# HSU-ANT/gstpeaq

Measured on AMD Instinct MI355X. Metric: 2048-sample stereo ref/test frame-pairs/sec (basic PEAQ, ear model -> MOVs -> ODG); ODG delta vs CPU ref, higher is better.
Workload: dtype f64

## Files before the change

### gstpeaq_amd/csrc/peaq_backend.hip

```cpp
#include <hip/hip_runtime.h>

#include <climits>
#include <cstdlib>

#include "peaq_device.h"
#include "peaq_kernels.h"
#include "peaq_wave.h"
#ifdef PEAQ_DEV_PROBES
#define PEAQ_DEV_TU_BACKEND
#include "dev_probes.inc"
#endif
#ifndef PEAQ_DEV_SPIN_INSTEAD_OF_BACKEND
#define PEAQ_DEV_SPIN_INSTEAD_OF_BACKEND(a, block, stream)
#endif

namespace peaq {

constexpr int kLdsBands = 128;
constexpr int kPaPad = 4, kPaStride = kPaPad + kLdsBands + 4;

constexpr int kAccLdsStride = 16;
struct LaneAcc {
  double* f;
  int mode, status;
// ... 299 lines not shown
            ld *
            (bt.pow(1. + div_fast(fmax(stest * e_test[s] - sref * e_ref[s], 0.), ethres + sref * e_ref[s] * beta), 0.23) - 1.);
        nl += t;
        terms[s] = t;
      }
    }
  }
  return nl;
}
template <int NB>
__device__ __forceinline__ double noise_loudness_total(double sum, double nl_min) {
  const double nl = sum * (24. / NB);
  return nl < nl_min ? 0. : nl;
}

template <int NB, int SLOTS, class TAB, bool TERMS = false>
__device__ __forceinline__ void mod_difference(const BandLane<NB, SLOTS>& bl, const TAB& bt,
                                               double lev_wt, const double (&mr)[SLOTS], const double (&mt)[SLOTS],
                                               const double (&loud_ref)[SLOTS], double& d1, double& d2, double& wt,
                                               double (*terms)[SLOTS] = nullptr) {
  double a1 = 0., a2 = 0., aw = 0.;
#pragma unroll
  for (int s = 0; s < SLOTS; ++s) {
    if (TERMS) terms[0][s] = terms[1][s] = terms[2][s] = 0.;
    if (bl.valid(s)) {
      const double diff = fabs(mr[s] - mt[s]);
      if (!TERMS) {
        a1 += div_fast(diff, 1. + mr[s]);
        a2 += div_fast((mt[s] >= mr[s] ? 1. : .1) * diff, 0.01 + mr[s]);
        aw += div_fast(loud_ref[s], loud_ref[s] + lev_wt * bt.noise_pow03(bl.band(s)));
      } else {
        a1 += terms[0][s] = div_fast(diff, 1. + mr[s]);
        a2 += terms[1][s] = div_fast((mt[s] >= mr[s] ? 1. : .1) * diff, 0.01 + mr[s]);
        aw += terms[2][s] = div_fast(loud_ref[s], loud_ref[s] + lev_wt * bt.noise_pow03(bl.band(s)));
      }
    }
  }
  double unused;
  wave_sum4(a1, a2, aw, 0., d1, d2, wt, unused);
}

__device__ __forceinline__ uint32_t wave_uniform(uint32_t x) { return (uint32_t)__builtin_amdgcn_readfirstlane((int)x); }
template <bool FB>
struct PointWalk {
  PointSnap* row;
  uint32_t n_min, interval;
  int n_points, k;
  uint32_t due;
  __device__ __forceinline__ static uint32_t count(uint32_t a) {
    return FB ? a / kFbFrame : a >= (uint32_t)kFrame ? (a - kFrame) / kHop + 1 : 0u;
  }
  __device__ __forceinline__ void set_due(int k1) {
    k = k1;
    if (k1 >= n_points) {
      due = UINT_MAX;
      return;
    }
    const uint64_t t = (uint64_t)(k1 + 1) * interval;
    due = count(t < n_min ? (uint32_t)t : n_min);
  }
  __device__ __forceinline__ void init(const PointArgs& p, unsigned pair, uint32_t c0) {
    row = p.snap + (size_t)pair * p.n_points;
    const uint32_t nr = p.n_ref ? p.n_ref[pair] : p.n_uniform, nt = p.n_test ? p.n_test[pair] : p.n_uniform;
    n_min = nr < nt ? nr : nt;
    interval = p.interval;
    n_points = p.n_points;
    const uint64_t thr = FB ? (uint64_t)kFbFrame * (c0 + 1ull) : (uint64_t)kFrame + (uint64_t)kHop * c0;
    const uint64_t k0 = n_min < thr ? (uint64_t)n_points : (thr + interval - 1) / interval - 1;
    set_due(k0 < (uint64_t)n_points ? (int)k0 : n_points);
  }
  __device__ __forceinline__ PointSnap* take(uint32_t c) {
    if (wave_uniform(due) != c) return nullptr;
    const int k1 = (int)wave_uniform((uint32_t)k);
    const uint64_t r = reinterpret_cast<uint64_t>(row);
    PointSnap* sp = reinterpret_cast<PointSnap*>(((uint64_t)wave_uniform((uint32_t)(r >> 32)) << 32) |
                                                 wave_uniform((uint32_t)r)) + k1;
    set_due(k1 + 1);
    return sp;
  }
};

template <int NB, class ARGS>
__device__ __forceinline__ void band_store(const ARGS& bnd, uint32_t bit, size_t cell, int lane, double v0, double v1) {
  if (!(bnd.planes & bit)) return;
  const unsigned n_planes = __builtin_popcount(bnd.planes), slot = __builtin_popcount(bnd.planes & (bit - 1u));
  char* __restrict__ row = reinterpret_cast<char*>(bnd.bands + (cell * n_planes + slot) * band_row(NB));
  unsigned off = (unsigned)lane * 16u;
  asm volatile("" : "+v"(off));
  if (2 * lane < NB) *reinterpret_cast<double2*>(row + off) = make_double2(v0, v1);
}

__device__ __forceinline__ void fb_band_store(const FbBandArgs& bnd, uint32_t bit, size_t row0, int lane, double v) {
  if (!(bnd.planes & bit)) return;
  const unsigned slot = __builtin_popcount(bnd.planes & (bit - 1u));
  char* __restrict__ row = reinterpret_cast<char*>(bnd.bands + (row0 + slot) * kFbBands);
  unsigned off = (unsigned)lane * 8u;
  asm volatile("" : "+v"(off));
  if (lane < kFbBands) *reinterpret_cast<double*>(row + off) = v;
}

__device__ __forceinline__ double fb_summary_pick(int lane, double band_value, double den) {
  return lane < kFbBands ? band_value : lane == kFbBands ? den : 0.;
}
__device__ __forceinline__ void fb_summary_add(double* entry, bool own, double v) {
  if (own) *entry += v;
}
__device__ __forceinline__ void fb_summary_copy(double* dst, const double* src, bool own) {
  if (!own) return;
#pragma unroll
  for (int k = 0; k < kFbSumRows; ++k) {
    asm volatile("" ::: "memory");
    dst[k * kFbSumRow] = src[k * kFbSumRow];
  }
}

__device__ __forceinline__ void summary_add(double* row, bool own, double v0, double v1) {
  if (!own) return;
  double2* __restrict__ p = reinterpret_cast<double2*>(row);
  double2 v = *p;
  v.x += v0;
  v.y += v1;
  *p = v;
}
__device__ __forceinline__ void summary_max(double* row, bool own, bool last, double v0, double v1) {
  if (!own) return;
  double2* __restrict__ p = reinterpret_cast<double2*>(row);
  double2 v = *p;
  if (v0 > v.x) v.x = v0;
  if (last)
    v.y += 1.;
  else if (v1 > v.y)
    v.y = v1;
  *p = v;
}
template <int R, int ROW>
__device__ __forceinline__ void summary_copy(double* dst, const double* src, bool own) {
  if (!own) return;
#pragma unroll
  for (int k = 0; k < R; ++k) {
    asm volatile("" ::: "memory");
    *reinterpret_cast<double2*>(dst + k * ROW) = *reinterpret_cast<const double2*>(src + k * ROW);
  }
}

enum { MB_BW_REF, MB_BW_TEST, MB_NMR, MB_WINMOD, MB_ADB, MB_EHS, MB_AVGMOD1, MB_AVGMOD2, MB_NOISELOUD, MB_MFPD,
       MB_RELDIST };
enum { MA_RMSMOD, MA_NLASYM, MA_SEGNMR, MA_EHS, MA_LINDIST };

struct BackendShared {
  double pa[2][2][kPaStride];
  double pc[2][kLdsBands];
  double qc[2][kLdsBands];
  double acc[2][kAccFields][kAccLdsStride];
  double energy[2];
  int gate[2];
};

template <int NB, bool ADV, bool DBG = false>
__global__ __launch_bounds__(128, 3) void backend_kernel(BackendArgs a) {
  constexpr bool PTS = false, TRC = false, BND = false, PBD = false, SUM = false;
  constexpr SummaryArgs sum{};
  constexpr PointArgs pts{};
  constexpr TraceArgs trc{};
  constexpr BandArgs bnd{};
  constexpr PatternBandArgs pbd{};
#include "peaq_backend_fft.inc"
}
template <int NB, bool ADV>
__global__ __launch_bounds__(128, 3) void backend_points_kernel(BackendArgs a, PointArgs pts) {
  constexpr bool DBG = false, PTS = true, TRC = false, BND = false, PBD = false, SUM = false;
  constexpr SummaryArgs sum{};
  constexpr TraceArgs trc{};
  constexpr BandArgs bnd{};
  constexpr PatternBandArgs pbd{};
#include "peaq_backend_fft.inc"
}
template <int NB, bool ADV>
__global__ __launch_bounds__(128, 3) void backend_trace_kernel(BackendArgs a, TraceArgs trc) {
  constexpr bool DBG = false, PTS = false, TRC = true, BND = false, PBD = false, SUM = false;
  constexpr SummaryArgs sum{};
  constexpr PointArgs pts{};
  constexpr BandArgs bnd{};
  constexpr PatternBandArgs pbd{};
#include "peaq_backend_fft.inc"
}
template <int NB, bool ADV>
__global__ __launch_bounds__(128, 3) void backend_bands_kernel(BackendArgs a, BandArgs bnd) {
  constexpr bool DBG = false, PTS = false, TRC = false, BND = true, PBD = false, SUM = false;
  constexpr SummaryArgs sum{};
  constexpr PointArgs pts{};
  constexpr TraceArgs trc{};
  constexpr PatternBandArgs pbd{};
#include "peaq_backend_fft.inc"
}
template <int NB, bool ADV>
__global__ __launch_bounds__(128, 3) void backend_pattern_bands_kernel(BackendArgs a, PatternBandArgs pbd) {
  static_assert(!ADV, "the 55-band path has no pattern layer");
  constexpr bool DBG = false, PTS = false, TRC = false, BND = false, PBD = true, SUM = false;
  constexpr SummaryArgs sum{};
  constexpr PointArgs pts{};
  constexpr TraceArgs trc{};
  constexpr BandArgs bnd{};
#include "peaq_backend_fft.inc"
}
template <int NB, bool ADV>
__global__ __launch_bounds__(128, 3) void backend_summary_kernel(BackendArgs a, SummaryArgs sum) {
  constexpr bool DBG = false, PTS = false, TRC = false, BND = false, PBD = false, SUM = true;
  constexpr PointArgs pts{};
  constexpr TraceArgs trc{};
  constexpr BandArgs bnd{};
  constexpr PatternBandArgs pbd{};
#include "peaq_backend_fft.inc"
}

hipError_t launch_backend(const BackendArgs& a, unsigned n_pairs, hipStream_t stream, const RunOutputs& out) {
  if (n_pairs == 0) return hipSuccess;
  const dim3 block(64 * a.channels);
  PEAQ_DEV_SPIN_INSTEAD_OF_BACKEND(a, block, stream)
  const bool pts = out.has_pts(), trc = out.has_trc(), bnd = out.has_bnd(), pbd = out.has_pbd(), sum = out.has_sum();
  const int alone = bnd + pbd + sum;
  if (alone && (alone + pts + trc + (a.debug != nullptr) + (a.pair_frame0 != nullptr) > 1 || (pbd && a.advanced) ||
                (sum && a.pair_slot)))
    return hipErrorInvalidValue;
  if (out.has_win() && (!trc || alone || pts || a.debug || a.pair_frame0 || a.pair_slot || a.advanced))
    return hipErrorInvalidValue;
  if (sum && !a.advanced)
    hipLaunchKernelGGL((backend_summary_kernel<109, false>), dim3(n_pairs), block, 0, stream, a, out.sum);
  else if (sum)
    hipLaunchKernelGGL((backend_summary_kernel<55, true>), dim3(n_pairs), block, 0, stream, a, out.sum);
  else if (pbd)
    hipLaunchKernelGGL((backend_pattern_bands_kernel<109, false>), dim3(n_pairs), block, 0, stream, a, out.pbd);
  else if (bnd && !a.advanced)
    hipLaunchKernelGGL((backend_bands_kernel<109, false>), dim3(n_pairs), block, 0, stream, a, out.bnd);
  else if (bnd)
    hipLaunchKernelGGL((backend_bands_kernel<55, true>), dim3(n_pairs), block, 0, stream, a, out.bnd);
  else if (trc && !a.advanced)
    hipLaunchKernelGGL((backend_trace_kernel<109, false>), dim3(n_pairs), block, 0, stream, a, out.trc);
  else if (trc)
    hipLaunchKernelGGL((backend_trace_kernel<55, true>), dim3(n_pairs), block, 0, stream, a, out.trc);
  else if (pts && !a.advanced)
    hipLaunchKernelGGL((backend_points_kernel<109, false>), dim3(n_pairs), block, 0, stream, a, out.pts);
  else if (pts)
    hipLaunchKernelGGL((backend_points_kernel<55, true>), dim3(n_pairs), block, 0, stream, a, out.pts);
  else if (!a.advanced && a.debug)
    hipLaunchKernelGGL((backend_kernel<109, false, true>), dim3(n_pairs), block, 0, stream, a);
  else if (a.debug)
    hipLaunchKernelGGL((backend_kernel<55, true, true>), dim3(n_pairs), block, 0, stream, a);
  else if (!a.advanced)
    hipLaunchKernelGGL((backend_kernel<109, false>), dim3(n_pairs), block, 0, stream, a);
  else
    hipLaunchKernelGGL((backend_kernel<55, true>), dim3(n_pairs), block, 0, stream, a);
  return hipGetLastError();
}

struct FbBackendShared {
  double pa[2][2][kPaStride];
  double acc[2][kAccFields][kAccLdsStride];
  int gate[2];
};

template <bool DBG>
__global__ __launch_bounds__(128, 4) void fb_backend_kernel(FbBackendArgs a) {
  constexpr bool PTS = false, TRC = false, BND = false, FSUM = false;
  constexpr PointArgs pts{};
  constexpr TraceArgs trc{};
  constexpr FbBandArgs bnd{};
  constexpr FbSummaryArgs fsum{};
#include "peaq_backend_fb.inc"
}
__global__ __launch_bounds__(128, 4) void fb_backend_points_kernel(FbBackendArgs a, PointArgs pts) {
  constexpr bool DBG = false, PTS = true, TRC = false, BND = false, FSUM = false;
  constexpr TraceArgs trc{};
  constexpr FbBandArgs bnd{};
  constexpr FbSummaryArgs fsum{};
#include "peaq_backend_fb.inc"
}
__global__ __launch_bounds__(128, 4) void fb_backend_trace_kernel(FbBackendArgs a, TraceArgs trc) {
  constexpr bool DBG = false, PTS = false, TRC = true, BND = false, FSUM = false;
  constexpr PointArgs pts{};
  constexpr FbBandArgs bnd{};
  constexpr FbSummaryArgs fsum{};
#include "peaq_backend_fb.inc"
}
__global__ __launch_bounds__(128, 4) void fb_backend_bands_kernel(FbBackendArgs a, FbBandArgs bnd) {
  constexpr bool DBG = false, PTS = false, TRC = false, BND = true, FSUM = false;
  constexpr PointArgs pts{};
  constexpr TraceArgs trc{};
  constexpr FbSummaryArgs fsum{};
#include "peaq_backend_fb.inc"
}
__global__ __launch_bounds__(128, 4) void fb_band_summary_kernel(FbBackendArgs a, FbSummaryArgs fsum) {
  constexpr bool DBG = false, PTS = false, TRC = false, BND = false, FSUM = true;
  constexpr PointArgs pts{};
  constexpr TraceArgs trc{};
  constexpr FbBandArgs bnd{};
#include "peaq_backend_fb.inc"
}

hipError_t launch_fb_backend(const FbBackendArgs& a, unsigned n_pairs, hipStream_t stream, const RunOutputs& out) {
  if (n_pairs == 0) return hipSuccess;
  const bool pts = out.has_pts(), trc = out.has_trc(), bnd = out.has_fbnd(), fsum = out.has_fsum();
  if ((bnd || fsum) && (pts || trc || a.debug || a.windows || (bnd && fsum) || (fsum && out.has_sum())))
    return hipErrorInvalidValue;
  if (fsum)
    hipLaunchKernelGGL(fb_band_summary_kernel, dim3(n_pairs), dim3(64 * a.channels), 0, stream, a, out.fsum);
  else if (bnd)
    hipLaunchKernelGGL(fb_backend_bands_kernel, dim3(n_pairs), dim3(64 * a.channels), 0, stream, a, out.fbnd);
  else if (trc)
    hipLaunchKernelGGL(fb_backend_trace_kernel, dim3(n_pairs), dim3(64 * a.channels), 0, stream, a, out.trc);
  else if (pts)
    hipLaunchKernelGGL(fb_backend_points_kernel, dim3(n_pairs), dim3(64 * a.channels), 0, stream, a, out.pts);
  else if (a.debug)
    hipLaunchKernelGGL(fb_backend_kernel<true>, dim3(n_pairs), dim3(64 * a.channels), 0, stream, a);
  else
    hipLaunchKernelGGL(fb_backend_kernel<false>, dim3(n_pairs), dim3(64 * a.channels), 0, stream, a);
  return hipGetLastError();
}

__global__ void state_init_kernel(PairState* st, unsigned n_pairs) {
  const unsigned pair = blockIdx.x;
  if (pair >= n_pairs) return;
  PairState* ps = st + pair;
  double* raw = reinterpret_cast<double*>(ps);
  for (unsigned i = threadIdx.x; i < sizeof(PairState) / sizeof(double); i += blockDim.x) raw[i] = 0.;
  __syncthreads();
  if (threadIdx.x == 0) {
    ps->loudness_reached = UINT_MAX;
    for (int i = 0; i < kMaxAcc; ++i) ps->status[i] = kInit;
    for (int c = 0; c < 2; ++c)
      for (int i = 0; i < kMaxAcc; ++i) {
        ps->ch[c].acc[i][3] = ps->ch[c].acc[i][4] = ps->ch[c].acc[i][5] = __builtin_nan("");
      }
  }
}

hipError_t launch_state_init(PairState* state, int , unsigned n_pairs, hipStream_t stream) {
  if (n_pairs == 0) return hipSuccess;
  hipLaunchKernelGGL(state_init_kernel, dim3(n_pairs), dim3(256), 0, stream, state, n_pairs);
  return hipGetLastError();
}

static_assert(kInit == 0, "points_init_kernel writes status as zero");
__global__ void points_init_kernel(double* __restrict__ raw, size_t n_doubles) {
  const size_t i = (size_t)blockIdx.x * blockDim.x + threadIdx.x;
  if (i >= n_doubles) return;
  const unsigned j = (unsigned)(i % kSnapDoubles);
  double v = 0.;
  if (j >= (unsigned)kSnapAccHead) {
    const unsigned f = (j - kSnapAccHead) % kAccFields;
    if (f >= 3 && f <= 5) v = __builtin_nan("");
  }
  raw[i] = v;
}

hipError_t launch_points_init(PointSnap* snap, size_t n_snaps, hipStream_t stream) {
  if (n_snaps == 0) return hipSuccess;
  const size_t n = n_snaps * kSnapDoubles;
  hipLaunchKernelGGL(points_init_kernel, dim3((unsigned)((n + 255) / 256)), dim3(256), 0, stream,
                     reinterpret_cast<double*>(snap), n);
  return hipGetLastError();
// ... 129 lines not shown
```

### gstpeaq_amd/csrc/peaq_backend_fft.inc

```
  __shared__ BackendShared sh;
  __shared__ double sh_tab[T_COUNT * kBandStride];
  __shared__ __attribute__((aligned(16))) double sh_ltab[2 * kLogTabEntries + 2];
  constexpr int SLOTS = 2;
  const int lane = threadIdx.x & 63;
  const int chan = __builtin_amdgcn_readfirstlane(threadIdx.x >> 6);
  const int channels = a.channels;
  const unsigned pair = blockIdx.x;
  const BandLane<NB, SLOTS> bl{lane};
  {
    const BandTables* __restrict__ g = a.bands;
    const double* const src[T_COUNT] = {g->adapt_tc, g->ear_tc, g->threshold, g->loud_factor, g->exc_threshold,
                                        g->internal_noise, g->noise_pow03, g->mask_diff, g->inv_spread_norm,
                                        g->inv_spread_norm_pow03, g->ln_internal_noise, g->inv_window_count};
#pragma unroll
    for (int t = 0; t < T_COUNT; ++t)
      for (int i = threadIdx.x; i < kBandStride; i += blockDim.x) sh_tab[t * kBandStride + i] = src[t][i];
    for (int i = threadIdx.x; i < 2 * kLogTabEntries; i += blockDim.x) sh_ltab[i] = a.common->log_tab[i >> 1][i & 1];
  }
  LdsTabs bt{sh_tab, 0, a.bands->deriv_factor, sh_ltab};
  PairState* __restrict__ ps = a.state + (a.pair_slot ? a.pair_slot[pair] : pair);
  ChannelState* __restrict__ cs = &ps->ch[chan];

  unsigned f_begin, f_end;
  if (a.pair_frame0) {
    f_begin = a.pair_frame0[pair];
    f_end = f_begin + a.pair_nframes[pair];
  } else {
    const unsigned n_frames = a.n_frames ? a.n_frames[pair] : a.n_frames_uniform;
    f_begin = a.frame0;
    f_end = a.frame0 + a.frames_per_launch;
    if (f_end > n_frames) f_end = n_frames;
  }
  if (f_begin >= f_end) return;
  const bool clk_wave = a.clk && blockIdx.x == 0 && chan == 0;
  unsigned long long clk_s0 = 0, clk_w0 = 0;
  if (clk_wave) {
    clk_w0 = wall_clock64();
    clk_s0 = __builtin_readcyclecounter();
  }
  if (lane < kPaPad) sh.pa[chan][0][lane] = sh.pa[chan][1][lane] = 0.;
  __syncthreads();

  constexpr int SUM_R = band_summary_rows(ADV), SUM_ROW = band_row(NB);
  __shared__ __attribute__((aligned(16))) double sh_sum[SUM ? 2 * SUM_R * SUM_ROW : 2];
  const bool sum_own = SUM && 2 * lane < NB;
  const bool sum_last = SUM && 2 * lane + 1 == NB;
  auto sum_at = [&](double* base) -> double* {
    unsigned off = (unsigned)lane * 16u;
    asm volatile("" : "+v"(off));
    return reinterpret_cast<double*>(reinterpret_cast<char*>(base) + off);
  };
  auto sum_row = [&](int k) -> double* { return sum_at(sh_sum + (SUM ? (chan * SUM_R + k) * SUM_ROW : 0)); };
  auto sum_cell = [&](double* base) -> double* {
    return sum_at(base + ((size_t)pair * channels + chan) * (SUM_R * SUM_ROW));
  };
  int sum_st = kInit;
  if (SUM) {
    sum_st = __builtin_amdgcn_readfirstlane(ps->status[ADV ? (int)MA_SEGNMR : (int)MB_NMR]);
    summary_copy<SUM_R, SUM_ROW>(sum_row(0), sum_cell(sum.rows), sum_own);
  }

  double sm[2][SLOTS];
  double la[6][SLOTS];
  double mdr[3][SLOTS], mdt[3][SLOTS];
#pragma unroll
  for (int s = 0; s < SLOTS; ++s) {
    const int b = bl.band(s);
    sm[0][s] = cs->vec[kSmearRef][b < kBandStride ? b : 0];
    sm[1][s] = (BND || SUM) && ADV ? 0. : cs->vec[kSmearTest][b < kBandStride ? b : 0];
#pragma unroll
    for (int v = 0; v < 6; ++v) la[v][s] = cs->vec[kLaFiltRef + v][b < kBandStride ? b : 0];
#pragma unroll
    for (int v = 0; v < 3; ++v) {
      mdr[v][s] = cs->vec[kModPrevRef + v][b < kBandStride ? b : 0];
      mdt[v][s] = cs->vec[kModPrevTest + v][b < kBandStride ? b : 0];
    }
  }
  constexpr bool MDT_LDS = SUM && !ADV;
  __shared__ __attribute__((aligned(16))) double sh_mdt[MDT_LDS ? 2 * 3 * kLdsBands : 2];
  auto mdt_at = [&](int v) -> double2* {
    return reinterpret_cast<double2*>(sum_at(sh_mdt + (MDT_LDS ? (chan * 3 + v) * kLdsBands : 0)));
  };
  if (MDT_LDS) {
#pragma unroll
    for (int v = 0; v < 3; ++v) *mdt_at(v) = make_double2(mdt[v][0], mdt[v][1]);
    asm volatile("" ::: "memory");
  }
  LaneAcc acc;
  {
    const int i = lane < kMaxAcc ? lane : 0;
    acc.load(&sh.acc[chan][0][lane < kAccLdsStride ? lane : kAccLdsStride - 1], cs->acc[i], acc_mode(ADV, i),
             ps->status[i]);
  }
  unsigned loud_reached = ps->loudness_reached;
  __shared__ PointWalk<false> sh_pw[2];
  PointWalk<false>& pw = sh_pw[chan];
  if (PTS) pw.init(pts, pair, f_begin);
  __shared__ __attribute__((aligned(16))) double sh_trc[2][8];
  unsigned trc_full = 0;
  if (TRC) {
    const uint32_t nr = trc.n_ref ? trc.n_ref[pair] : trc.n_uniform, nt = trc.n_test ? trc.n_test[pair] : trc.n_uniform;
    trc_full = PointWalk<false>::count(nr < nt ? nr : nt);
    if (ADV && lane == 0) {
#pragma unroll
      for (int k = 2; k < 8; ++k) sh_trc[chan][k] = 0.;
    }
  }
  if (chan == 0 && lane == 0) {
    sh.energy[0] = ps->sig_energy;
    sh.energy[1] = ps->noise_energy;
  }
  for (unsigned frame = f_begin; frame < f_end; ++frame) {
    asm volatile("" : "+v"(bt.off));
    const double* __restrict__ rec0 =
        a.records + ((size_t)(pair * a.frames_per_launch + (frame - f_begin)) * channels) * kRecDoubles;
    const double* __restrict__ rec = rec0 + (size_t)chan * kRecDoubles;

    int fl_ref = (int)rec0[kRecFlagsRef], fl_test = (int)rec0[kRecFlagsTest];
    if (channels == 2) {
      fl_ref |= (int)rec0[kRecDoubles + kRecFlagsRef];
      fl_test |= (int)rec0[kRecDoubles + kRecFlagsTest];
    }
    const bool above = fl_ref & 1;
    const bool ehs_valid = ((fl_ref | fl_test) & 2) != 0;
    if (!ADV || lane == MA_SEGNMR || lane == MA_EHS) acc.set_tentative(!above);
    bool sum_cnt = false;
    if (SUM) {
      if (__builtin_amdgcn_readfirstlane((int)above)) {
        sum_st = kNormal;
      } else if (sum_st == kNormal) {
        summary_copy<SUM_R, SUM_ROW>(sum_cell(sum.saved), sum_row(0), sum_own);
        sum_st = kTentative;
      }
      sum_st = __builtin_amdgcn_readfirstlane(sum_st);
      sum_cnt = sum_st != kInit;
    }

    double ur[SLOTS], ut[SLOTS], lr[SLOTS], lt[SLOTS], nz[SLOTS];
    {
      const int b0 = bl.band(0);
      const int bb = b0 < kBandStride ? b0 : 0;
      const double2 v0 = *reinterpret_cast<const double2*>(rec + kRecRootRef + bb);
      const double2 v1 = *reinterpret_cast<const double2*>(rec + kRecRootTest + bb);
      const double2 v4 = *reinterpret_cast<const double2*>(rec + kRecNoise + bb);
      const double n0 = bt.at(T_ISN, bb), n1 = bt.at(T_ISN, bb + 1);
      const double m0 = bt.at(T_ISN03, bb), m1 = bt.at(T_ISN03, bb + 1);
      excitation_from_root(v0.x, n0, m0, ur[0], lr[0]);
      excitation_from_root(v0.y, n1, m1, ur[1], lr[1]);
      excitation_from_root(v1.x, n0, m0, ut[0], lt[0]);
      excitation_from_root(v1.y, n1, m1, ut[1], lt[1]);
      nz[0] = v4.x; nz[1] = v4.y;
    }
    if (PBD || (SUM && !ADV)) nz[0] = nz[1] = 0.;
    const size_t pbd_cell = PBD ? ((size_t)pair * pbd.frame_stride + frame) * channels + chan : 0;
    if (PBD) {
      band_store<NB>(pbd, kPatBandUnsmRef, pbd_cell, lane, ur[0], bl.valid(1) ? ur[1] : 0.);
      band_store<NB>(pbd, kPatBandUnsmTest, pbd_cell, lane, ut[0], bl.valid(1) ? ut[1] : 0.);
    }
    double nl_part = 0.;
    bool nl_open = false;
    double er[SLOTS], et[SLOTS];
#pragma unroll
    for (int s = 0; s < SLOTS; ++s) {
      const int b = bl.band(s) < kBandStride ? bl.band(s) : 0;
      const double ac = bt.ear_tc(b);
      if (SUM && !ADV)
        sm[0][s] = __builtin_fma(ac, sm[0][s], (1. - ac) * ur[s]);
      else
        sm[0][s] = ac * sm[0][s] + (1. - ac) * ur[s];
      er[s] = sm[0][s] > ur[s] ? sm[0][s] : ur[s];
      if (!ADV) {
        if (SUM)
          sm[1][s] = __builtin_fma(1. - ac, ut[s], ac * sm[1][s]);
        else
          sm[1][s] = ac * sm[1][s] + (1. - ac) * ut[s];
        et[s] = sm[1][s] > ut[s] ? sm[1][s] : ut[s];
      } else {
        et[s] = 0.;
      }
    }

    const size_t bnd_cell = BND ? ((size_t)pair * bnd.frame_stride + frame) * channels + chan : 0;
    if (BND) {
      band_store<NB>(bnd, kBandExcRef, bnd_cell, lane, er[0], bl.valid(1) ? er[1] : 0.);
      if (!ADV) band_store<NB>(bnd, kBandExcTest, bnd_cell, lane, et[0], bl.valid(1) ? et[1] : 0.);
    }
    if (PBD) {
      band_store<NB>(pbd, kPatBandExcRef, pbd_cell, lane, er[0], bl.valid(1) ? er[1] : 0.);
      band_store<NB>(pbd, kPatBandExcTest, pbd_cell, lane, et[0], bl.valid(1) ? et[1] : 0.);
    }
    if (SUM && sum_cnt) {
      summary_add(sum_row(kSumExcRef), sum_own, er[0], sum_last ? 1. : er[1]);
      if (!ADV) summary_add(sum_row(kSumExcTest), sum_own, et[0], sum_last ? 1. : et[1]);
    }

    double my_v = 0., my_w = 1.;
    bool my_hit = false;
    auto route = [&](int idx, double v, double w) {
      if (lane == idx) {
        my_v = v;
        my_w = w;
        my_hit = true;
      }
    };

    if (!ADV) {
      double ad_ref[SLOTS], ad_test[SLOTS], mr[SLOTS], mt[SLOTS];
      level_adapt<NB, SLOTS>(bl, bt, er, et, la, &sh.pa[chan][0][0], ad_ref, ad_test);
      modulation<NB, SLOTS>(bl, bt, lr, mdr, mr);
      if (MDT_LDS) {
        double m[3][SLOTS];
#pragma unroll
        for (int v = 0; v < 3; ++v) {
          const double2 t = *mdt_at(v);
          m[v][0] = t.x;
          m[v][1] = t.y;
        }
        modulation<NB, SLOTS, LdsTabs, true>(bl, bt, lt, m, mt);
#pragma unroll
        for (int v = 0; v < 3; ++v) *mdt_at(v) = make_double2(m[v][0], m[v][1]);
      } else {
        modulation<NB, SLOTS>(bl, bt, lt, mdt, mt);
      }
      if (PBD) {
        band_store<NB>(pbd, kPatBandAdaptRef, pbd_cell, lane, ad_ref[0], ad_ref[1]);
        band_store<NB>(pbd, kPatBandAdaptTest, pbd_cell, lane, ad_test[0], ad_test[1]);
        band_store<NB>(pbd, kPatBandModRef, pbd_cell, lane, mr[0], mr[1]);
        band_store<NB>(pbd, kPatBandModTest, pbd_cell, lane, mt[0], mt[1]);
        band_store<NB>(pbd, kPatBandAvgLoudRef, pbd_cell, lane, mdr[1][0], bl.valid(1) ? mdr[1][1] : 0.);
      }
      if (DBG) {
        double* __restrict__ d =
            a.debug + ((size_t)(pair * a.frames_per_launch + (frame - f_begin)) * channels + chan) * kDbgDoubles;
#pragma unroll
        for (int s = 0; s < SLOTS; ++s) {
          if (bl.valid(s)) {
            const int b = bl.band(s);
            d[kDbgExcRef + b] = er[s];
            d[kDbgExcTest + b] = et[s];
            d[kDbgAdaptRef + b] = ad_ref[s];
            d[kDbgAdaptTest + b] = ad_test[s];
            d[kDbgModRef + b] = mr[s];
            d[kDbgModTest + b] = mt[s];
            d[kDbgAvgLoudRef + b] = mdr[1][s];
            d[kDbgAvgLoudTest + b] = mdt[1][s];
          }
        }
      }
      if (loud_reached == UINT_MAX) {
        double n_ref, n_test;
        wave_sum2(total_loudness_part<NB, SLOTS>(bl, bt, er), total_loudness_part<NB, SLOTS>(bl, bt, et), n_ref, n_test);
        n_ref *= 24. / NB;
        n_test *= 24. / NB;
        if (lane == 0) sh.gate[chan] = (n_ref > 0.1 && n_test > 0.1);
        if (DBG && lane == 0) {
          double* __restrict__ d =
              a.debug + ((size_t)(pair * a.frames_per_launch + (frame - f_begin)) * channels + chan) * kDbgDoubles;
          d[kDbgLoudnessRef] = n_ref;
          d[kDbgLoudnessTest] = n_test;
        }
      }
      double bnd_x[SLOTS], bnd_q[SLOTS];
#pragma unroll
      for (int s = 0; s < SLOTS; ++s) {
        double pc = 0., qc = 0.;
        if (bl.valid(s)) {
          const double er_db = (10. * kInvLn10) * bt.log(er[s]);
          const double et_db = (10. * kInvLn10) * bt.log(et[s]);
          const double l = 0.3 * fmax(er_db, et_db) + 0.7 * et_db;
          const double l2 = l * l;
          const double sd = l > 0. ? 5.95072 * bt.exp(1.71332 * (1.8554663946857675 - bt.log(l))) + 9.01033e-11 * l2 * l2 +
                                         5.05622e-6 * l2 * l - 0.00102438 * l * l + 0.0550197 * l - 0.198719
                                   : 1e30;
          const double inv_sd = div_fast(1., sd);
          const double e = er_db - et_db;
          const double x = e * inv_sd, x2 = x * x;
          const double xb = er_db > et_db ? x2 * x2 : x2 * x2 * x2;
          pc = xb;
          qc = fabs(a.cfg.floor_steps ? floor(e) : trunc(e)) * inv_sd;
        }
        sh.pc[chan][bl.band(s)] = pc;
        sh.qc[chan][bl.band(s)] = qc;
        bnd_x[s] = pc;
        bnd_q[s] = qc;
      }
      if (BND) {
        band_store<NB>(bnd, kBandDetect, bnd_cell, lane, bnd_x[0], bnd_x[1]);
        band_store<NB>(bnd, kBandSteps, bnd_cell, lane, bnd_q[0], bnd_q[1]);
      }
      __syncthreads();
      if (loud_reached == UINT_MAX) {
        const int g = sh.gate[0] | (channels == 2 ? sh.gate[1] : 0);
        if (g) loud_reached = frame;
      }
      double* __restrict__ dmov =
          DBG ? a.debug + ((size_t)(pair * a.frames_per_launch + (frame - f_begin)) * channels + chan) * kDbgDoubles + kDbgMov
              : nullptr;
      if (DBG || TRC || PBD || frame >= 24) {
        double d1, d2, wt;
        if (PBD) {
          double md_t[3][SLOTS];
          mod_difference<NB, SLOTS, LdsTabs, true>(bl, bt, 100., mr, mt, mdr[1], d1, d2, wt, md_t);
          band_store<NB>(pbd, kPatBandModDiff1, pbd_cell, lane, md_t[0][0], md_t[0][1]);
          band_store<NB>(pbd, kPatBandModDiff2, pbd_cell, lane, md_t[1][0], md_t[1][1]);
          band_store<NB>(pbd, kPatBandModWt, pbd_cell, lane, md_t[2][0], md_t[2][1]);
        } else if (SUM) {
          double md_t[3][SLOTS];
          mod_difference<NB, SLOTS, LdsTabs, true>(bl, bt, 100., mr, mt, mdr[1], d1, d2, wt, md_t);
          if (sum_cnt) {
            summary_add(sum_row(kSumModDiff1), sum_own, wt * md_t[0][0], sum_last ? wt : wt * md_t[0][1]);
            summary_add(sum_row(kSumModDiff2), sum_own, wt * md_t[1][0], sum_last ? wt : wt * md_t[1][1]);
          }
        } else {
          mod_difference<NB, SLOTS>(bl, bt, 100., mr, mt, mdr[1], d1, d2, wt);
        }
        d1 *= 100. / NB;
        d2 *= 100. / NB;
        if (frame >= 24) {
          route(MB_AVGMOD1, d1, wt);
          route(MB_AVGMOD2, d2, wt);
          route(MB_WINMOD, d1, 1.);
        }
        if (DBG && lane == 0) {
          dmov[0] = d1;
          dmov[1] = d2;
          dmov[2] = wt;
        }
        if (TRC && lane == 0) {
          sh_trc[chan][0] = d1;
          sh_trc[chan][1] = d2;
          sh_trc[chan][2] = wt;
        }
      }
      nl_open = DBG || TRC || PBD || (frame >= 24 && frame - 3 >= loud_reached);
      if (PBD) {
        double nl_t[SLOTS];
        nl_part = noise_loudness_part<NB, SLOTS, LdsTabs, LEAD_OWN, true>(bl, bt, 1.5, 0.15, 0.5, mr, mt, ad_ref, ad_test,
                                                                          nullptr, nl_t);
        band_store<NB>(pbd, kPatBandNoiseLoud, pbd_cell, lane, nl_t[0], nl_t[1]);
      } else if (SUM && nl_open) {
        double nl_t[SLOTS];
        nl_part = noise_loudness_part<NB, SLOTS, LdsTabs, LEAD_OWN, true>(bl, bt, 1.5, 0.15, 0.5, mr, mt, ad_ref, ad_test,
                                                                          nullptr, nl_t);
        if (sum_cnt) summary_add(sum_row(kSumNoiseLoud), sum_own, nl_t[0], sum_last ? 1. : nl_t[1]);
      } else if (nl_open) {
        nl_part = noise_loudness_part<NB, SLOTS>(bl, bt, 1.5, 0.15, 0.5, mr, mt, ad_ref, ad_test);
      }
      {
        const double bw_ref = rec[kRecBwRef];
        if (bw_ref > 346.) {
          route(MB_BW_REF, bw_ref, 1.);
          route(MB_BW_TEST, rec[kRecBwTest], 1.);
        }
      }
    }
    {
      double nsum = 0., nmax = 0.;
      double bnd_r[SLOTS] = {0., 0.};
      if (PBD || (SUM && !ADV)) {
        const int b0 = bl.band(0);
        const double2 v4 = *reinterpret_cast<const double2*>(rec + kRecNoise + (b0 < kBandStride ? b0 : 0));
        nz[0] = v4.x; nz[1] = v4.y;
      }
#pragma unroll
      for (int s = 0; s < SLOTS; ++s) {
        if (bl.valid(s)) {
          const double r = div_fast(nz[s] * bt.mask_diff(bl.band(s)), er[s]);
          nsum += r;
          if (r > nmax) nmax = r;
          bnd_r[s] = r;
        }
      }
      if (BND) band_store<NB>(bnd, kBandNmr, bnd_cell, lane, bnd_r[0], bnd_r[1]);
      if (SUM && sum_cnt) {
        summary_add(sum_row(kSumNmrSum), sum_own, bnd_r[0], sum_last ? 1. : bnd_r[1]);
        summary_max(sum_row(kSumNmrMax), sum_own, sum_last, bnd_r[0], bnd_r[1]);
        summary_add(sum_row(kSumNmrDisturbed), sum_own, bnd_r[0] > 1.41253754462275 ? 1. : 0.,
                    sum_last || bnd_r[1] > 1.41253754462275 ? 1. : 0.);
      }
      double xsum = 0., qsum = 0.;
      if (!ADV && chan == 0) {
#pragma unroll
        for (int s = 0; s < SLOTS; ++s) {
          if (bl.valid(s)) {
            const int b = bl.band(s);
            double x = fmax(sh.pc[0][b], 0.), q = sh.qc[0][b];
            if (channels == 2) {
              if (sh.pc[1][b] > x) x = sh.pc[1][b];
              if (sh.qc[1][b] > q) q = sh.qc[1][b];
            }
            xsum += x;
            qsum += q;
          }
        }
      }
      double nl_sum;
      if (!ADV)
        wave_sum4(nsum, nl_part, qsum, xsum, nsum, nl_sum, qsum, xsum);
      else
        nsum = wave_sum(nsum);
      nsum /= NB;
      const bool disturbed = __any(nmax > 1.41253754462275);
      if (DBG || TRC) nmax = wave_max(nmax);
      if (!ADV && nl_open) {
        const double nl = noise_loudness_total<NB>(nl_sum, 0.);
        if (frame >= 24 && frame - 3 >= loud_reached) route(MB_NOISELOUD, nl, 1.);
        if (DBG && lane == 0)
          a.debug[((size_t)(pair * a.frames_per_launch + (frame - f_begin)) * channels + chan) * kDbgDoubles + kDbgMov + 3] = nl;
        if (TRC && lane == 0) sh_trc[chan][3] = nl;
      }
      if (DBG && lane == 0) {
        double* __restrict__ d =
            a.debug + ((size_t)(pair * a.frames_per_launch + (frame - f_begin)) * channels + chan) * kDbgDoubles + kDbgMov;
        d[4] = nsum;
        d[5] = nmax;
      }
      if (TRC && !ADV && lane == 0) {
        sh_trc[chan][4] = nsum;
        sh_trc[chan][5] = nmax;
      }
      if (!ADV) {
        route(MB_NMR, nsum, 1.);
        route(MB_RELDIST, disturbed ? 1. : 0., 1.);
      } else {
        const double seg = (10. * kInvLn10) * log_pos(nsum);
        route(MA_SEGNMR, seg, 1.);
        if (DBG && lane == 0)
          a.debug[((size_t)(pair * a.frames_per_launch + (frame - f_begin)) * channels + chan) * kDbgDoubles + kDbgMov + 3] = seg;
        if (TRC && lane == 0) {
          sh_trc[chan][0] = seg;
          sh_trc[chan][1] = nsum;
        }
      }
      if (!ADV && chan == 0) {
        const double p_bin = 1. - bt.exp(-kLn2 * xsum);
        if (DBG && lane == 0) {
          double* __restrict__ d =
              a.debug + ((size_t)(pair * a.frames_per_launch + (frame - f_begin)) * channels) * kDbgDoubles + kDbgMov;
          d[6] = p_bin;
          d[7] = qsum;
        }
        if (TRC && lane == 0) {
          sh_trc[0][6] = p_bin;
          sh_trc[0][7] = qsum;
        }
        if (p_bin > 0.5) route(MB_ADB, qsum, 1.);
        route(MB_MFPD, p_bin, 1.);
      }
    }
    if (ehs_valid) {
      route(ADV ? MA_EHS : MB_EHS, 1000. * rec[kRecEhs], 1.);
    }
    if (chan == 0 && lane == 0) {
      sh.energy[0] += rec0[kRecSigE] + (channels == 2 ? rec0[kRecDoubles + kRecSigE] : 0.);
      sh.energy[1] += rec0[kRecNoiseE] + (channels == 2 ? rec0[kRecDoubles + kRecNoiseE] : 0.);
    }
    if (my_hit) acc.add(my_v, my_w);
    if (PTS) {
      while (PointSnap* __restrict__ sp = pw.take(frame + 1)) {
        if (lane < kMaxAcc && (!ADV || lane == MA_SEGNMR || lane == MA_EHS)) {
#pragma unroll
          for (int k = 0; k < kAccFields; ++k) sp->acc[chan][lane][k] = acc.at(k);
          if (chan == 0) sp->status[lane] = acc.status;
        }
        if (chan == 0 && lane == 0) {
          sp->frames = frame + 1;
          sp->sig_energy = sh.energy[0];
          sp->noise_energy = sh.energy[1];
        }
      }
    }
    if (TRC && lane == 0) {
      const double2* __restrict__ s = reinterpret_cast<const double2*>(sh_trc[chan]);
      double2* __restrict__ o = reinterpret_cast<double2*>(trc.frames + (size_t)pair * trc.frame_stride + frame);
#pragma unroll
      for (int k = 0; k < 3; ++k) o[3 * chan + k] = s[k];
      if (chan == 0) {
        const uint32_t fl = (above ? kTraceAbove : 0u) | (!ADV && frame >= 24 ? kTraceModOpen : 0u) |
                            (!ADV && frame >= 24 && frame - 3 >= loud_reached ? kTraceLoudOpen : 0u) |
                            (frame >= trc_full ? kTraceFlush : 0u);
        if (channels == 1) {
#pragma unroll
          for (int k = 3; k < 6; ++k) o[k] = make_double2(0., 0.);
        }
        o[6] = s[3];
        o[7] = make_double2(__hiloint2double((int)frame, (int)fl), 0.);
      }
    }
    if (!ADV) __syncthreads();
  }

  if (MDT_LDS) {
    asm volatile("" ::: "memory");
#pragma unroll
    for (int v = 0; v < 3; ++v) {
      const double2 t = *mdt_at(v);
      mdt[v][0] = t.x;
      mdt[v][1] = t.y;
    }
  }
#pragma unroll
  for (int s = 0; s < SLOTS; ++s) {
    const int b = bl.band(s);
    if (b < kBandStride) {
      cs->vec[kSmearRef][b] = sm[0][s];
      if (!((BND || SUM) && ADV)) cs->vec[kSmearTest][b] = sm[1][s];
      if (!ADV) {
#pragma unroll
        for (int v = 0; v < 6; ++v) cs->vec[kLaFiltRef + v][b] = la[v][s];
#pragma unroll
        for (int v = 0; v < 3; ++v) {
          cs->vec[kModPrevRef + v][b] = mdr[v][s];
          cs->vec[kModPrevTest + v][b] = mdt[v][s];
        }
      }
    }
  }
  if (lane < kMaxAcc) {
    if (!ADV || lane == MA_SEGNMR || lane == MA_EHS) {
      acc.store(cs->acc[lane]);
      if (chan == 0) ps->status[lane] = acc.status;
    }
  }
  if (chan == 0 && lane == 0) {
    ps->frame_counter = f_end;
    if (!ADV) ps->loudness_reached = loud_reached;
    ps->sig_energy = sh.energy[0];
    ps->noise_energy = sh.energy[1];
  }
  if (clk_wave && lane == 0) {
    a.clk[0] += __builtin_readcyclecounter() - clk_s0;
    a.clk[1] += wall_clock64() - clk_w0;
  }
  if (SUM) summary_copy<SUM_R, SUM_ROW>(sum_cell(sum.rows), sum_row(0), sum_own);
```

### gstpeaq_amd/csrc/peaq_device.h

```cpp
#pragma once

#include <stdint.h>

namespace peaq {

constexpr int kFrame      = 2048;
constexpr int kHop        = 1024;
constexpr int kBins       = 1025;
constexpr int kBandStride = 112;
constexpr int kFbFrame    = 192;
constexpr int kFbBands    = 40;
constexpr int kFbRing     = 1456;
constexpr int kFbTaps     = 11;
constexpr double kBackMask[6] = {0x1.6518acf1cfa3cp-7, 0x1.4d2ceb622adf4p-5, 0x1.4d2ceb622adf3p-4,
                                 0x1.f3c36113404ebp-4, 0x1.36db60930de4ep-3, 0x1.4d2ceb622adf1p-3};
constexpr int kFbCentre = 729;
constexpr int kMfTiles = 3;
constexpr int kMfD0[kMfTiles]    = {2, 470, 677};
constexpr int kMfSteps[kMfTiles] = {182, 65, 14};
constexpr int kMfBase[kMfTiles]  = {0, 182, 247};
constexpr int kMfTotalSteps = 261;
constexpr int kHfBlocks[kMfTiles] = {23, 9, 2};
constexpr int kHfBase[kMfTiles]   = {0, 23, 32};
constexpr int kHfD1[kMfTiles]     = {1, 465, 673};
constexpr int kHfD2[kMfTiles]     = {2, 466, 674};
constexpr int kHfTotalBlocks = 34;
enum { HF_RE_HI_1, HF_RE_LO_1, HF_IM_HI_1, HF_IM_LO_1, HF_RE_HI_2, HF_RE_LO_2, HF_NIM_HI_2, HF_NIM_LO_2, HF_OPERANDS };
constexpr int kBsBands  = 24;
constexpr int kBsPairs  = kBsBands / 2;
constexpr int kBsChains = kBsBands * 3;
constexpr int kBsHistOrg = 8;
constexpr int kBsHist   = kBsHistOrg + 48;
constexpr int bs_row(int sub, int ty) { return ty < 6 ? (ty & 1) * 6 + 3 * sub + (ty >> 1) : 12 + 2 * (ty - 6) + sub; }
constexpr int kBsSeg = 9;
constexpr int kMfdBand0 = 24;
constexpr int kMfdD0    = 611;
constexpr int kMfdSteps = 30;

struct CommonTables {
  double hann_lane[64][4];
  double ear_w2[kBins];
  double tw_re[kFrame];
  double tw_im[kFrame];
  double tw_lane[8][64][2];
  double ear_w2_pair[8][64][2];
  double ehs_window[256];
  double ehs_window_centred[256];
  double log_tab[130][2];
  double exp_tab[64];
};
constexpr int kLogTabEntries = 129;
constexpr int kExpTabEntries = 64;
constexpr int kLogTabFold = 54;

struct BandTables {
  int    bands;
  int    step;
  double delta_z;
  double dz02;
  double aLe;
  double deriv_factor;
  double fc[kBandStride];
  double internal_noise[kBandStride];
  double noise_pow03[kBandStride];
  double ear_tc[kBandStride];
  double adapt_tc[kBandStride];
  double exc_threshold[kBandStride];
  double threshold[kBandStride];
  double loud_factor[kBandStride];
  double ln_internal_noise[kBandStride];
  double inv_window_count[kBandStride];
  int    lo[kBandStride], hi[kBandStride];
  double wlo[kBandStride], whi[kBandStride];
  double ln_aUC[kBandStride];
  double gIL[kBandStride];
  double inv_spread_norm[kBandStride];
  double inv_spread_norm_pow03[kBandStride];
  double mask_diff[kBandStride];
};

struct FbTables {
  int    flen[kFbBands];
  int    delay[kFbBands];
  int    coef_off[kFbBands];
  double back_mask[6];
  double h_re[12000];
  double h_im[12000];
  double mf_re[kMfTotalSteps * 64];
  double mf_im[kMfTotalSteps * 64];
  float  mf_re_f[kMfTotalSteps * 64];
  float  mf_im_f[kMfTotalSteps * 64];
  unsigned short hf[kHfTotalBlocks][HF_OPERANDS][64][8];
  double hf_unscale[kMfTiles * 16];
  int    bs_col_head[kBsPairs];
  int    bs_off_enter[kBsBands];
  int    bs_col_left[kBsBands];
  int    bs_left_q0[kBsBands];
  int    bs_left_g[kBsBands][2];
  int    bs_whole[kBsBands];
  double bs_coef[kBsPairs][8][64];
  double bs_left[kBsBands][32][2];
  double bs_rot[kBsChains][2][2];
  double bs_pow[kBsChains][64][2];
  int    bs_seg_s[kBsBands];
  double bs_seg[kBsPairs][6][64][2];
  double mfd_re[kMfdSteps * 64];
  double mfd_im[kMfdSteps * 64];
  double log_tab[130][2];
};

struct Settings {
  int swap_mod_patts = 1;
  int centre_ehs_window = 0;
  int ehs_dc_before_window = 1;
  int floor_steps = 0;
  int clamp_movs = 0;
  int swap_slope = 0;
};

constexpr int kRecRootRef   = 0 * kBandStride;
constexpr int kRecRootTest  = 1 * kBandStride;
constexpr int kRecNoise     = 2 * kBandStride;
constexpr int kRecScalars   = 3 * kBandStride;
constexpr int kRecBwRef     = kRecScalars + 0;
constexpr int kRecBwTest    = kRecScalars + 1;
constexpr int kRecEhs       = kRecScalars + 2;
constexpr int kRecFlagsRef  = kRecScalars + 3;
constexpr int kRecFlagsTest = kRecScalars + 4;
constexpr int kRecSigE      = kRecScalars + 5;
constexpr int kRecNoiseE    = kRecScalars + 6;
constexpr int kRecDoubles   = 352;

#if defined(__HIPCC__)
__host__ __device__
#endif
inline void excitation_from_root(double root, double inv_norm, double inv_norm_pow03, double& unsm, double& loud) {
  const double r1 = root * root, e2 = r1 * r1;
  unsm = e2 * e2 * r1 * inv_norm;
  loud = r1 * root * inv_norm_pow03;
}

constexpr int kPubUnsmRef   = 0 * kBandStride;
constexpr int kPubUnsmTest  = 1 * kBandStride;
constexpr int kPubLoudRef   = 2 * kBandStride;
constexpr int kPubLoudTest  = 3 * kBandStride;
constexpr int kPubNoise     = 4 * kBandStride;
constexpr int kPubScalars   = 5 * kBandStride;
constexpr int kPubDoubles   = 576;

constexpr int kDbgExcRef       = 0 * kBandStride;
constexpr int kDbgExcTest      = 1 * kBandStride;
constexpr int kDbgAdaptRef     = 2 * kBandStride;
constexpr int kDbgAdaptTest    = 3 * kBandStride;
constexpr int kDbgModRef       = 4 * kBandStride;
constexpr int kDbgModTest      = 5 * kBandStride;
constexpr int kDbgAvgLoudRef   = 6 * kBandStride;
constexpr int kDbgAvgLoudTest  = 7 * kBandStride;
constexpr int kDbgLoudnessRef  = 8 * kBandStride;
constexpr int kDbgLoudnessTest = 8 * kBandStride + 1;
constexpr int kDbgMov          = 8 * kBandStride + 8;
constexpr int kDbgDoubles      = 8 * kBandStride + 16;

constexpr int kDbgFbDoubles = 8;

constexpr int kFbRecUnsmRef  = 0;
constexpr int kFbRecUnsmTest = 40;
constexpr int kFbRecExcRef   = 80;
constexpr int kFbRecExcTest  = 120;
constexpr int kFbRecFlags    = 160;
constexpr int kFbRecDoubles  = 168;

constexpr int kAccFields = 12;
constexpr int kMaxAcc    = 11;

enum AccMode { kAvg = 0, kAvgLog, kRms, kRmsAsym, kAvgWindow, kFilteredMax, kAdb };
enum AccStatus { kInit = 0, kNormal, kTentative };

enum StateVec {
  kSmearRef = 0, kSmearTest,
  kLaFiltRef, kLaFiltTest, kLaNum, kLaDen, kLaPcRef, kLaPcTest,
  kModPrevRef, kModLoudRef, kModDLoudRef,
  kModPrevTest, kModLoudTest, kModDLoudTest,
  kStateVecs
};

struct ChannelState {
  double vec[kStateVecs][kBandStride];
  double acc[kMaxAcc][kAccFields];
};

struct PairState {
  uint32_t frame_counter;
  uint32_t fb_counter;
  uint32_t loudness_reached;
  uint32_t pad0;
  int32_t  status[kMaxAcc];
  int32_t  pad1;
  double   sig_energy;
  double   noise_energy;
  ChannelState ch[2];
};

struct PointSnap {
  uint32_t frames;
  uint32_t fb_blocks;
  int32_t  status[kMaxAcc];
  int32_t  pad;
  double   sig_energy;
  double   noise_energy;
  double   acc[2][kMaxAcc][kAccFields];
};
constexpr int kSnapDoubles = sizeof(PointSnap) / sizeof(double);
constexpr int kSnapAccHead = (int)(sizeof(PointSnap) - sizeof(double) * 2 * kMaxAcc * kAccFields) / (int)sizeof(double);
static_assert(sizeof(PointSnap) % sizeof(double) == 0, "PointSnap is filled as doubles");

struct FbSignalState {
  double hp[6];
  double cu[kFbBands];
  double e0_hist[kFbBands][kFbTaps];
  double excitation[kFbBands];
  double ring[kFbRing];
  double peak_slot[3][2];
  double peak_last;
  double bs_hist[kBsBands][6][kBsHist];
};

}
```

Measured before the change: 31.48 million.

## Hoist per-frame record loads, gather scalars via lanes, prefetch next record

Each frame's band loads and per-channel scalar fields are now issued at the top of the loop. The scalars are fetched once into eight lanes and broadcast with readlane, replacing scattered scalar loads and the LDS energy accumulator. The signal and noise energy sums now live in registers. In the plain backend kernel, channel 0 touches every 128-byte line of the next frame's record as a prefetch, kept alive by an asm constraint. This is meant to hide global load latency in the serial frame loop, at the cost of extra loads and register pressure.

```diff
diff --git a/gstpeaq_amd/csrc/peaq_backend.hip b/gstpeaq_amd/csrc/peaq_backend.hip
--- a/gstpeaq_amd/csrc/peaq_backend.hip
+++ b/gstpeaq_amd/csrc/peaq_backend.hip
@@ -475,13 +475,17 @@
   double pc[2][kLdsBands];
   double qc[2][kLdsBands];
   double acc[2][kAccFields][kAccLdsStride];
-  double energy[2];
   int gate[2];
 };
 
+#ifdef PEAQ_BE_NO_WARM
+constexpr bool kBackendWarm = false;
+#else
+constexpr bool kBackendWarm = true;
+#endif
 template <int NB, bool ADV, bool DBG = false>
 __global__ __launch_bounds__(128, 3) void backend_kernel(BackendArgs a) {
-  constexpr bool PTS = false, TRC = false, BND = false, PBD = false, SUM = false;
+  constexpr bool PTS = false, TRC = false, BND = false, PBD = false, SUM = false, WARM = kBackendWarm && !DBG;
   constexpr SummaryArgs sum{};
   constexpr PointArgs pts{};
   constexpr TraceArgs trc{};
@@ -491,7 +495,7 @@
 }
 template <int NB, bool ADV>
 __global__ __launch_bounds__(128, 3) void backend_points_kernel(BackendArgs a, PointArgs pts) {
-  constexpr bool DBG = false, PTS = true, TRC = false, BND = false, PBD = false, SUM = false;
+  constexpr bool DBG = false, PTS = true, TRC = false, BND = false, PBD = false, SUM = false, WARM = false;
   constexpr SummaryArgs sum{};
   constexpr TraceArgs trc{};
   constexpr BandArgs bnd{};
@@ -500,7 +504,7 @@
 }
 template <int NB, bool ADV>
 __global__ __launch_bounds__(128, 3) void backend_trace_kernel(BackendArgs a, TraceArgs trc) {
-  constexpr bool DBG = false, PTS = false, TRC = true, BND = false, PBD = false, SUM = false;
+  constexpr bool DBG = false, PTS = false, TRC = true, BND = false, PBD = false, SUM = false, WARM = false;
   constexpr SummaryArgs sum{};
   constexpr PointArgs pts{};
   constexpr BandArgs bnd{};
@@ -509,7 +513,7 @@
 }
 template <int NB, bool ADV>
 __global__ __launch_bounds__(128, 3) void backend_bands_kernel(BackendArgs a, BandArgs bnd) {
-  constexpr bool DBG = false, PTS = false, TRC = false, BND = true, PBD = false, SUM = false;
+  constexpr bool DBG = false, PTS = false, TRC = false, BND = true, PBD = false, SUM = false, WARM = false;
   constexpr SummaryArgs sum{};
   constexpr PointArgs pts{};
   constexpr TraceArgs trc{};
@@ -519,7 +523,7 @@
 template <int NB, bool ADV>
 __global__ __launch_bounds__(128, 3) void backend_pattern_bands_kernel(BackendArgs a, PatternBandArgs pbd) {
   static_assert(!ADV, "the 55-band path has no pattern layer");
-  constexpr bool DBG = false, PTS = false, TRC = false, BND = false, PBD = true, SUM = false;
+  constexpr bool DBG = false, PTS = false, TRC = false, BND = false, PBD = true, SUM = false, WARM = false;
   constexpr SummaryArgs sum{};
   constexpr PointArgs pts{};
   constexpr TraceArgs trc{};
@@ -528,7 +532,7 @@
 }
 template <int NB, bool ADV>
 __global__ __launch_bounds__(128, 3) void backend_summary_kernel(BackendArgs a, SummaryArgs sum) {
-  constexpr bool DBG = false, PTS = false, TRC = false, BND = false, PBD = false, SUM = true;
+  constexpr bool DBG = false, PTS = false, TRC = false, BND = false, PBD = false, SUM = true, WARM = false;
   constexpr PointArgs pts{};
   constexpr TraceArgs trc{};
   constexpr BandArgs bnd{};
diff --git a/gstpeaq_amd/csrc/peaq_backend_fft.inc b/gstpeaq_amd/csrc/peaq_backend_fft.inc
--- a/gstpeaq_amd/csrc/peaq_backend_fft.inc
+++ b/gstpeaq_amd/csrc/peaq_backend_fft.inc
@@ -106,9 +106,10 @@
       for (int k = 2; k < 8; ++k) sh_trc[chan][k] = 0.;
     }
   }
-  if (chan == 0 && lane == 0) {
-    sh.energy[0] = ps->sig_energy;
-    sh.energy[1] = ps->noise_energy;
+  double e_sig = 0., e_noise = 0.;
+  if (chan == 0) {
+    e_sig = ps->sig_energy;
+    e_noise = ps->noise_energy;
   }
   for (unsigned frame = f_begin; frame < f_end; ++frame) {
     asm volatile("" : "+v"(bt.off));
@@ -116,10 +117,31 @@
         a.records + ((size_t)(pair * a.frames_per_launch + (frame - f_begin)) * channels) * kRecDoubles;
     const double* __restrict__ rec = rec0 + (size_t)chan * kRecDoubles;
 
-    int fl_ref = (int)rec0[kRecFlagsRef], fl_test = (int)rec0[kRecFlagsTest];
-    if (channels == 2) {
-      fl_ref |= (int)rec0[kRecDoubles + kRecFlagsRef];
-      fl_test |= (int)rec0[kRecDoubles + kRecFlagsTest];
+    const int bb = bl.band(0) < kBandStride ? bl.band(0) : 0;
+    const double2 v_root_ref = *reinterpret_cast<const double2*>(rec + kRecRootRef + bb);
+    const double2 v_root_test = *reinterpret_cast<const double2*>(rec + kRecRootTest + bb);
+    const double2 v_noise = *reinterpret_cast<const double2*>(rec + kRecNoise + bb);
+    double sc = 0.;
+    if (lane < kRecScalarsUsed || (channels == 2 && lane >= 8 && lane < 8 + kRecScalarsUsed))
+      sc = rec0[(lane < 8 ? kRecScalars : kRecDoubles + kRecScalars - 8) + lane];
+    unsigned warm_keep = 0;
+    if (WARM) {
+      const bool warm = chan == 0 && frame + 1 < f_end && lane < (kRecDoubles * 8 / 128) * channels;
+      const char* next = reinterpret_cast<const char*>(rec0 + channels * kRecDoubles) + (unsigned)lane * 128u;
+      warm_keep = *reinterpret_cast<const unsigned*>(warm ? next : reinterpret_cast<const char*>(rec0));
+    }
+
+    const int sc_i = (int)sc;
+    const int fl_ref = __builtin_amdgcn_readlane(sc_i, kRecFlagsRef - kRecScalars) |
+                       __builtin_amdgcn_readlane(sc_i, 8 + kRecFlagsRef - kRecScalars);
+    const int fl_test = __builtin_amdgcn_readlane(sc_i, kRecFlagsTest - kRecScalars) |
+                        __builtin_amdgcn_readlane(sc_i, 8 + kRecFlagsTest - kRecScalars);
+    const double bw_ref = lane_value_d(sc, 8 * chan + kRecBwRef - kRecScalars);
+    const double bw_test = lane_value_d(sc, 8 * chan + kRecBwTest - kRecScalars);
+    const double ehs = lane_value_d(sc, 8 * chan + kRecEhs - kRecScalars);
+    if (chan == 0) {
+      e_sig += read_lane<kRecSigE - kRecScalars>(sc) + read_lane<8 + kRecSigE - kRecScalars>(sc);
+      e_noise += read_lane<kRecNoiseE - kRecScalars>(sc) + read_lane<8 + kRecNoiseE - kRecScalars>(sc);
     }
     const bool above = fl_ref & 1;
     const bool ehs_valid = ((fl_ref | fl_test) & 2) != 0;
@@ -138,11 +160,7 @@
 
     double ur[SLOTS], ut[SLOTS], lr[SLOTS], lt[SLOTS], nz[SLOTS];
     {
-      const int b0 = bl.band(0);
-      const int bb = b0 < kBandStride ? b0 : 0;
-      const double2 v0 = *reinterpret_cast<const double2*>(rec + kRecRootRef + bb);
-      const double2 v1 = *reinterpret_cast<const double2*>(rec + kRecRootTest + bb);
-      const double2 v4 = *reinterpret_cast<const double2*>(rec + kRecNoise + bb);
+      const double2 v0 = v_root_ref, v1 = v_root_test, v4 = v_noise;
       const double n0 = bt.at(T_ISN, bb), n1 = bt.at(T_ISN, bb + 1);
       const double m0 = bt.at(T_ISN03, bb), m1 = bt.at(T_ISN03, bb + 1);
       excitation_from_root(v0.x, n0, m0, ur[0], lr[0]);
@@ -346,12 +364,9 @@
       } else if (nl_open) {
         nl_part = noise_loudness_part<NB, SLOTS>(bl, bt, 1.5, 0.15, 0.5, mr, mt, ad_ref, ad_test);
       }
-      {
-        const double bw_ref = rec[kRecBwRef];
-        if (bw_ref > 346.) {
-          route(MB_BW_REF, bw_ref, 1.);
-          route(MB_BW_TEST, rec[kRecBwTest], 1.);
-        }
+      if (bw_ref > 346.) {
+        route(MB_BW_REF, bw_ref, 1.);
+        route(MB_BW_TEST, bw_test, 1.);
       }
     }
     {
@@ -449,11 +464,7 @@
       }
     }
     if (ehs_valid) {
-      route(ADV ? MA_EHS : MB_EHS, 1000. * rec[kRecEhs], 1.);
-    }
-    if (chan == 0 && lane == 0) {
-      sh.energy[0] += rec0[kRecSigE] + (channels == 2 ? rec0[kRecDoubles + kRecSigE] : 0.);
-      sh.energy[1] += rec0[kRecNoiseE] + (channels == 2 ? rec0[kRecDoubles + kRecNoiseE] : 0.);
+      route(ADV ? MA_EHS : MB_EHS, 1000. * ehs, 1.);
     }
     if (my_hit) acc.add(my_v, my_w);
     if (PTS) {
@@ -465,8 +476,8 @@
         }
         if (chan == 0 && lane == 0) {
           sp->frames = frame + 1;
-          sp->sig_energy = sh.energy[0];
-          sp->noise_energy = sh.energy[1];
+          sp->sig_energy = e_sig;
+          sp->noise_energy = e_noise;
         }
       }
     }
@@ -487,6 +498,7 @@
         o[7] = make_double2(__hiloint2double((int)frame, (int)fl), 0.);
       }
     }
+    if (WARM) asm volatile("" ::"v"(warm_keep));
     if (!ADV) __syncthreads();
   }
 
@@ -525,8 +537,8 @@
   if (chan == 0 && lane == 0) {
     ps->frame_counter = f_end;
     if (!ADV) ps->loudness_reached = loud_reached;
-    ps->sig_energy = sh.energy[0];
-    ps->noise_energy = sh.energy[1];
+    ps->sig_energy = e_sig;
+    ps->noise_energy = e_noise;
   }
   if (clk_wave && lane == 0) {
     a.clk[0] += __builtin_readcyclecounter() - clk_s0;
diff --git a/gstpeaq_amd/csrc/peaq_device.h b/gstpeaq_amd/csrc/peaq_device.h
--- a/gstpeaq_amd/csrc/peaq_device.h
+++ b/gstpeaq_amd/csrc/peaq_device.h
@@ -129,7 +129,10 @@
 constexpr int kRecFlagsTest = kRecScalars + 4;
 constexpr int kRecSigE      = kRecScalars + 5;
 constexpr int kRecNoiseE    = kRecScalars + 6;
+constexpr int kRecScalarsUsed = 7;
 constexpr int kRecDoubles   = 352;
+static_assert(kRecScalarsUsed <= 8 && (kRecScalars * 8) % 128 == 0 && (kRecDoubles * 8) % 128 == 0,
+              "the back end gathers a channel's scalars into eight lanes, and warms a record line by line");
 
 #if defined(__HIPCC__)
 __host__ __device__
```

Result: faster. 32.44 million, median of 6 (+3.0%).
